# cvxopt/cvxopt

Hardware: NVIDIA H100
Metric: kkt_factor_solve_gflops_fp64 (higher is better)
Workload: dtype f64

## Files before the change

cvxopt_b200/_lib.py:

```python
import ctypes as C
import os

_HERE = os.path.dirname(os.path.abspath(__file__))
LIB_PATH = os.path.join(_HERE, "libcvxopt_b200.so")

HOST, DEVICE = 0, 1
E_ARG, E_CUDA, E_NOMEM, E_NOGPU, E_UNSUP = -1, -2, -3, -4, -5

c_double_p = C.POINTER(C.c_double)
c_int_p = C.POINTER(C.c_int)


class Dims(C.Structure):
    _fields_ = [("mnl", C.c_int), ("ml", C.c_int), ("nq", C.c_int), ("q", c_int_p),
                ("ns", C.c_int), ("s", c_int_p)]


class Scaling(C.Structure):
    _fields_ = [(name, C.c_void_p) for name in
                ("dnl", "dnli", "d", "di", "v", "beta", "r", "rti")]


class SblockArgs(C.Structure):
    _fields_ = ([("nblk", C.c_int), ("orders", C.c_void_p), ("m", C.c_longlong), ("L", C.c_longlong),
# ... 25 lines not shown
    "cvxb_kkt_destroy": (None, [C.c_void_p]),
    "cvxb_kkt_reset": (C.c_int, [C.c_void_p]),
    "cvxb_kkt_set_method": (C.c_int, [C.c_void_p, C.c_int, C.c_double]),
    "cvxb_kkt_set_H": (C.c_int, [C.c_void_p, C.c_void_p, C.c_int, C.c_int]),
    "cvxb_kkt_factor": (C.c_int, [C.c_void_p, C.POINTER(Scaling), C.c_void_p, C.c_int,
                                  C.c_void_p, C.c_int, C.c_int, C.c_int]),
    "cvxb_kkt_solve": (C.c_int, [C.c_void_p, C.c_void_p, C.c_void_p, C.c_void_p, C.c_int]),
    "cvxb_kkt_get_L": (C.c_int, [C.c_void_p, C.c_void_p, C.c_int]),
    "cvxb_kkt_last_ms": (C.c_int, [C.c_void_p, c_double_p, c_double_p]),
    "cvxb_kkt_timer_start": (C.c_int, [C.c_void_p]),
    "cvxb_kkt_timer_stop": (C.c_int, [C.c_void_p, c_double_p]),
    "cvxb_kkt_trace": (C.c_int, [C.c_void_p, C.c_void_p, C.c_int]),
    "cvxb_kkt_last_breakdown": (C.c_int, [C.c_void_p, c_double_p]),
    "cvxb_kkt_syrk_mma_ms": (C.c_int, [C.c_void_p, c_double_p]),
    "cvxb_kkt_syrk_path": (C.c_int, [C.c_void_p]),
    "cvxb_kkt_qr_passes": (C.c_int, [C.c_void_p]),
    "cvxb_kkt_gemv_G": (C.c_int, [C.c_void_p, C.c_void_p, C.c_void_p, C.c_double, C.c_double,
                                  C.c_int, C.c_int]),
    "cvxb_kkt_gemv_A": (C.c_int, [C.c_void_p, C.c_void_p, C.c_void_p, C.c_double, C.c_double,
                                  C.c_int, C.c_int]),
    "cvxb_kkt_symv_H": (C.c_int, [C.c_void_p, C.c_void_p, C.c_void_p, C.c_double, C.c_double,
                                  C.c_int]),
    "cvxb_scale": (C.c_int, [C.c_void_p, C.c_int, C.c_int, C.POINTER(Dims), C.POINTER(Scaling),
                             C.c_int, C.c_int, C.c_int]),
    "cvxb_scale2": (C.c_int, [C.c_void_p, C.c_void_p, C.POINTER(Dims), C.c_int, C.c_int]),
    "cvxb_pack": (C.c_int, [C.c_void_p, C.c_void_p, C.POINTER(Dims), C.c_int]),
    "cvxb_pack2": (C.c_int, [C.c_void_p, C.c_int, C.c_int, C.POINTER(Dims), C.c_int]),
    "cvxb_unpack": (C.c_int, [C.c_void_p, C.c_void_p, C.POINTER(Dims), C.c_int]),
    "cvxb_symm": (C.c_int, [C.c_void_p, C.c_int, C.c_int]),
    "cvxb_sprod": (C.c_int, [C.c_void_p, C.c_void_p, C.POINTER(Dims), C.c_int, C.c_int]),
# ... 123 lines not shown
```

cvxopt_b200/csrc/chol.cu:

```cuda
#include "common.cuh"
#include <cstdlib>

namespace cvxb {

namespace {

constexpr int PB = 8;
constexpr int SP = 12;
constexpr int LDM = NB + 4;
constexpr int POTF2_SMEM = (NB * LDM + NB * SP + 4 * 80) * 8;
constexpr int kGroup = 4;

template <int PAT>
__device__ __forceinline__ void sym_update(double (&acc)[4][8][2], const double *Ma, const double *Mb) {
#pragma unroll 2
    for (int kk = 0; kk < NB / 4; ++kk) {
        double a[4], bfr[8];
#pragma unroll
        for (int cf = 0; cf < 4; ++cf) a[cf] = -Ma[cf * 8 + kk * 4 * LDM];
#pragma unroll
        for (int rf = 0; rf < 8; ++rf) bfr[rf] = Mb[rf * 8 + kk * 4 * LDM];
#pragma unroll
        for (int mf = 0; mf < 2; ++mf)
#pragma unroll
// ... 442 lines not shown
}

std::atomic<int> g_trsv_epoch{0};

__global__ void __launch_bounds__(256)
transpose_panel_kernel(const double *__restrict__ W, long long ldw, int rows, double *__restrict__ WT, long long ldt) {
    __shared__ double t[32][33];
    const int r0 = blockIdx.x * 32, k0 = blockIdx.y * 32, tx = threadIdx.x, ty = threadIdx.y;
#pragma unroll
    for (int i = ty; i < 32; i += 8)
        if (r0 + tx < rows) t[i][tx] = W[r0 + tx + (long long)(k0 + i) * ldw];
    __syncthreads();
#pragma unroll
    for (int i = ty; i < 32; i += 8)
        if (r0 + i < rows) WT[k0 + tx + (long long)(r0 + i) * ldt] = t[tx][i];
}

}

int chol_work_create(CholWork &w) {
    int least = 0, greatest = 0;
    CVXB_CUDA(cudaDeviceGetStreamPriorityRange(&least, &greatest));
    CVXB_CUDA(cudaStreamCreateWithPriority(&w.panel_stream, cudaStreamNonBlocking, greatest));
    CVXB_CUDA(cudaStreamCreateWithPriority(&w.trsm_stream, cudaStreamNonBlocking, greatest));
    CVXB_CUDA(cudaStreamCreateWithPriority(&w.update_stream, cudaStreamNonBlocking, least));
    CVXB_CUDA(cudaStreamCreateWithPriority(&w.near_stream, cudaStreamNonBlocking, greatest));
    CVXB_CUDA(cudaEventCreateWithFlags(&w.ev_end_t, cudaEventDisableTiming));
    CVXB_CUDA(cudaEventCreateWithFlags(&w.ev_end_n, cudaEventDisableTiming));
    CVXB_CUDA(cudaEventCreateWithFlags(&w.ev_start, cudaEventDisableTiming));
    CVXB_CUDA(cudaEventCreateWithFlags(&w.ev_end_p, cudaEventDisableTiming));
// ... 8 lines not shown
    CVXB_CUDA(cudaFuncSetAttribute(trsv_kernel<true, true>, cudaFuncAttributeMaxDynamicSharedMemorySize, TRSV_SMEM));
    CVXB_CUDA(cudaFuncSetAttribute(trsv_kernel<true, false>, cudaFuncAttributeMaxDynamicSharedMemorySize, TRSV_SMEM));
    CVXB_CUDA(cudaFuncSetAttribute(trsv_kernel<false, true>, cudaFuncAttributeMaxDynamicSharedMemorySize, TRSV_SMEM));
    CVXB_CUDA(cudaFuncSetAttribute(trsv_kernel<false, false>, cudaFuncAttributeMaxDynamicSharedMemorySize, TRSV_SMEM));
    return 0;
}

CholWork::~CholWork() {
    for (cudaStream_t s : {panel_stream, update_stream, trsm_stream, near_stream}) if (s) cudaStreamDestroy(s);
    for (auto &g : graphs) if (g.exec) cudaGraphExecDestroy(g.exec);
    for (cudaEvent_t e : {ev_end_t, ev_end_n, ev_start, ev_end_p, ev_end_u}) if (e) cudaEventDestroy(e);
    for (auto *v : {&ev_dg, &ev_tr, &ev_c0, &ev_na, &ev_nb, &ev_n})
        for (cudaEvent_t e : *v) cudaEventDestroy(e);
}

static int potrf_enqueue(int n, double *A, int lda, double *inv, CholWork &w, cudaStream_t st) {
    if (n <= 0) return 0;
    const int nblk = (n + NB - 1) / NB;
    if (w.panel_rows < n) {
        for (auto &g : w.graphs) if (g.exec) cudaGraphExecDestroy(g.exec);
        w.graphs.clear();
        for (DevBuf<double> &pb : w.panel) pb.reset();
        for (DevBuf<double> &gb : w.group) gb.reset();
        const int rows = (n + 1) & ~1;
        for (DevBuf<double> &pb : w.panel) CVXB_TRY(pb.alloc((size_t)rows * NB));
        for (DevBuf<double> &gb : w.group) CVXB_TRY(gb.alloc((size_t)rows * kGroup * NB));
        w.panel_rows = rows;
    }
    while ((int)w.ev_dg.size() < nblk) {
        cudaEvent_t e[6];
        for (int i = 0; i < 6; ++i) CVXB_CUDA(cudaEventCreateWithFlags(&e[i], cudaEventDisableTiming));
        w.ev_dg.push_back(e[0]); w.ev_tr.push_back(e[1]); w.ev_c0.push_back(e[2]);
        w.ev_na.push_back(e[3]); w.ev_nb.push_back(e[4]); w.ev_n.push_back(e[5]);
    }
    if (getenv("CVXB_TRACE") && !w.trace.p) CVXB_TRY(w.trace.alloc(8 * 4096));
    unsigned long long *trace = w.trace.p;
    if (trace) CVXB_CUDA(cudaMemsetAsync(trace, 0, 8 * 4096 * sizeof(unsigned long long), st));
    const int ldw = w.panel_rows;
    const int ldg = kGroup * NB;
    cudaStream_t D = w.panel_stream, T = w.trsm_stream, U = w.update_stream, N = w.near_stream;
    CVXB_CUDA(cudaMemsetAsync(w.d_info.p, 0, sizeof(int), st));
    CVXB_CUDA(cudaEventRecord(w.ev_start, st));
    for (cudaStream_t s : {D, T, U, N}) CVXB_CUDA(cudaStreamWaitEvent(s, w.ev_start, 0));
    auto update = [&](int lo, int hi, const double *X, int ldx, bool kmajor, int K, unsigned long long *tr,
                      cudaStream_t s) -> int {
        double *Acc = A + (long long)lo * NB * (1 + (long long)lda);
        GemmDesc u;
        u.M = n - lo * NB; u.N = (hi * NB < n ? hi * NB : n) - lo * NB; u.K = K;
        u.X = X; u.ldx = ldx; u.x_kmajor = kmajor;
        u.Y = X; u.ldy = ldx; u.y_kmajor = kmajor;
        u.D = Acc; u.ldd = lda; u.C = Acc; u.ldc = lda;
        u.alpha = -1.0; u.beta = 1.0; u.lower_only = true;
        u.trace = tr;
        return dmma_gemm(u, s);
    };
    auto wait_col = [&](cudaStream_t s, int c) -> int {
        const int p = c - 2, g0 = kGroup * (c / kGroup);
        if (p < 0) return 0;
        if (p >= g0) CVXB_CUDA(cudaStreamWaitEvent(s, w.ev_na[p], 0));
        if (g0 > 0) CVXB_CUDA(cudaStreamWaitEvent(s, w.ev_nb[p < g0 - 1 ? p : g0 - 1], 0));
        return 0;
    };
    for (int jb = 0; jb < nblk; ++jb) {
        const int j = jb * NB;
        const int wj = (n - j < NB) ? (n - j) : NB;
        const int m = n - j - wj;
        double *Ajj = A + j + (long long)j * lda;
        double *invj = inv + (long long)jb * NB * NB;
        double *invTj = inv + (long long)(nblk + jb) * NB * NB;
        double *Wp = w.panel[jb & 1].p;
// ... 64 lines not shown
                Wp + (gq - jb - 1) * NB, ldw, rows, Wg + s * NB, ldg);
            count_launch();
            CVXB_LAUNCH_CHECK();
        }
        CVXB_CUDA(cudaEventRecord(w.ev_n[jb], N));
        if (gq < nblk) {
            CVXB_CUDA(cudaStreamWaitEvent(U, w.ev_n[jb], 0));
            const int lo = gq > jb + 2 ? gq : jb + 2, hi = gq + kGroup < nblk ? gq + kGroup : nblk;
            if (lo < hi) CVXB_TRY(update(lo, hi, Wg + s * NB + (long long)(lo - gq) * NB * ldg, ldg, true, NB, tr_near, U));
            CVXB_CUDA(cudaEventRecord(w.ev_nb[jb], U));
            if (s == kGroup - 1 && gq + kGroup < nblk)
                CVXB_TRY(update(gq + kGroup, nblk, Wg + (long long)kGroup * NB * ldg, ldg, true, kGroup * NB,
                                trace ? trace + 8 * 2048 + 8 * jb + 5 : nullptr, U));
        }
    }
    CVXB_CUDA(cudaEventRecord(w.ev_end_p, D));
    CVXB_CUDA(cudaEventRecord(w.ev_end_u, U));
    CVXB_CUDA(cudaEventRecord(w.ev_end_t, T));
    CVXB_CUDA(cudaEventRecord(w.ev_end_n, N));
    for (cudaEvent_t e : {w.ev_end_p, w.ev_end_u, w.ev_end_t, w.ev_end_n}) CVXB_CUDA(cudaStreamWaitEvent(st, e, 0));
    return 0;
}

int potrf_lower(int n, double *A, int lda, double *inv, CholWork &w, cudaStream_t st) {
    if (n <= 0) return 0;
    if (w.graph_failed || n > 4096) return potrf_enqueue(n, A, lda, inv, w, st);
    CholWork::GraphEntry *ent = nullptr;
    for (auto &g : w.graphs)
        if (g.n == n && g.A == A && g.lda == lda && g.inv == inv) { ent = &g; break; }
    if (ent && ent->exec) {
// ... 128 lines not shown
```

cvxopt_b200/csrc/common.cuh:

```cuda
#pragma once
#include <cuda_runtime.h>
#include <cstdio>
#include <cstdint>
#include <cstring>
#include <string>
#include <vector>
#include <atomic>
#include <mutex>
#include "../../include/cvxopt_b200.h"

namespace cvxb {

void set_error(const char *fmt, ...);
extern std::atomic<unsigned long long> g_launches;
inline void count_launch(int n = 1) { g_launches.fetch_add((unsigned long long)n, std::memory_order_relaxed); }

struct DeviceOnce {
    std::atomic<unsigned long long> done{0};
    unsigned long long pending() {
        int d = 0;
        cudaGetDevice(&d);
        const unsigned long long bit = 1ull << (d & 63);
        return (done.load(std::memory_order_acquire) & bit) ? 0ull : bit;
    }
// ... 226 lines not shown

struct GemmDesc {
    int M = 0, N = 0, K = 0;
    const double *X = nullptr; int ldx = 0; bool x_kmajor = false;
    const double *Y = nullptr; int ldy = 0; bool y_kmajor = false;
    const double *w = nullptr;
    const double *D = nullptr; int ldd = 0;
    double *C = nullptr; int ldc = 0;
    double alpha = 1.0, beta = 0.0;
    bool lower_only = false;
    int ct_begin = 0, ct_end = 1 << 30;
    int batch = 1;
    long long sX = 0, sY = 0, sW = 0, sD = 0, sC = 0;
    double *splitk_ws = nullptr;
    unsigned long long *trace = nullptr;
};
int dmma_gemm(const GemmDesc &g, cudaStream_t st);
size_t dmma_gemm_splitk_ws_doubles();
int dmma_gemm_tile_cols();

size_t ozaki_workspace_bytes(int n, int m, int S);
int ozaki_mode();
bool ozaki_use(int mode, int n, int m, DevBuf<char> &work);
void ozaki_time_mma(cudaEvent_t a, cudaEvent_t b);
int ozaki_syrk(int n, int m, const double *A, long long lda, const double *d, const double *D,
               long long ldd, double beta, double *C, long long ldc, int S, int layout, void *work,
               cudaStream_t st);

struct CholWork {
    cudaStream_t panel_stream = nullptr;
// ... 5 lines not shown
    DevBuf<unsigned long long> trace;
    struct GraphEntry {
        int n = 0, lda = 0, launches = 0;
        const void *A = nullptr, *inv = nullptr;
        cudaGraphExec_t exec = nullptr;
    };
    std::vector<GraphEntry> graphs;
    bool graph_failed = false;
    cudaEvent_t ev_start = nullptr, ev_end_p = nullptr, ev_end_u = nullptr;
    DevBuf<int> d_info;
    DevBuf<int> d_flags;
    DevBuf<double> splitk_ws;
    DevBuf<double> panel[2];
    DevBuf<double> group[2];
    int panel_rows = 0;
    ~CholWork();
};
int chol_work_create(CholWork &w);
int potrf_lower(int n, double *A, int lda, double *inv, CholWork &w, cudaStream_t st);
int potrs_lower(int n, const double *L, int ldl, const double *inv, double *b, CholWork &w,
                cudaStream_t st, int batch = 1, long long sL = 0, long long sInv = 0,
                long long sb = 0);
int trsv_lower(int n, const double *L, int ldl, const double *inv, double *b, bool trans,
               CholWork &w, cudaStream_t st, int batch = 1, long long sL = 0, long long sInv = 0,
               long long sb = 0);
int potrf_lower_batched(int n, double *A, int lda, long long sA, double *inv, long long sInv,
                        int batch, int *d_info, double *panel, int ldw, cudaStream_t st);
int trsm_lower_left(int n, const double *L, long long ldl, const double *inv, double *B, long long ldb, int ncols,
                    cudaStream_t st, int batch = 1, long long sL = 0, long long sInv = 0, long long sB = 0);

int check_device(int device);

struct CallCtx {
    cudaStream_t st = nullptr;
// ... 7 lines not shown
```

cvxopt_b200/csrc/gemm_dmma.cu:

```cuda
#include "common.cuh"
#include <cuda.h>
#include <cudaTypedefs.h>

namespace cvxb {

namespace {

constexpr int BR = 128, BC = 64, BK = 16, STAGES = 3;
constexpr int THREADS = 128;
constexpr int SK = BK + 4;
constexpr int SMX = BR + 4;
constexpr int SMY = BC + 4;
constexpr int X_STAGE = BR * SK;
constexpr int Y_STAGE = BC * SK;
constexpr int STAGE_DOUBLES = X_STAGE + Y_STAGE + BK;
constexpr int SMEM_BYTES = STAGES * STAGE_DOUBLES * 8;
constexpr int TILE_ELEMS = BR * BC;
constexpr int CTAS_PER_WAVE = 2 * kNumSMs;
constexpr int SPLITK_WS_TILES = 4 * CTAS_PER_WAVE;

struct KParams {
    int M, N, K;
    const double *X; long long ldx;
    const double *Y; long long ldy;
// ... 1 lines not shown
    const double *D; long long ldd;
    double *C; long long ldc;
    double alpha, beta;
    int lower_only;
    int ct_begin, ct_end;
    int nTr;
    long long sX, sY, sW, sD, sC;
    int full_tiles;
    int S;
    int kchunk;
    double *ws;
    int vec_c;
    int stagger_ns;
    unsigned long long *trace;
    int band;
};

__device__ __host__ __forceinline__ int first_tr(int tc, int tcols) { return (tc * tcols) / BR; }

template <int TC>
__device__ __forceinline__ void decode_tile(const KParams &p, int t, int &tr, int &tc) {
    int c = p.ct_begin;
    if (p.lower_only && p.band > 0) {
        int cb_end;
        while (true) {
            cb_end = min(c + p.band, p.ct_end);
            int cnt = 0;
            for (int cc = c; cc < cb_end; ++cc) cnt += max(0, p.nTr - first_tr(cc, TC));
            if (t < cnt) break;
            t -= cnt;
// ... 357 lines not shown
    }
}

constexpr int TB = 128;
constexpr int T_STAGES = 6;
constexpr int T_CONSUMERS = 8;
constexpr int T_THREADS = 32 * (T_CONSUMERS + 4);
constexpr int T_REGS_PRODUCER = 40, T_REGS_CONSUMER = 232;
constexpr int T_PANEL = TB * BK;
constexpr int T_SMEM = T_STAGES * (2 * T_PANEL + BK) * 8 + 2 * T_STAGES * 8 + 1024;
constexpr int T_TILE_ELEMS = TB * TB;
constexpr int T_WS_TILES = 4 * kNumSMs;

__global__ void __launch_bounds__(T_THREADS, 1)
syrk_tma_kernel(const KParams p, const __grid_constant__ CUtensorMap tmX, const __grid_constant__ CUtensorMap tmY,
                const __grid_constant__ CUtensorMap tmW) {
    extern __shared__ unsigned char t_smem_raw[];
    double *sm = reinterpret_cast<double *>(t_smem_raw + ((1024u - (smem_u32(t_smem_raw) & 1023u)) & 1023u));
    double *sw = sm + T_STAGES * 2 * T_PANEL;
    uint64_t *full = reinterpret_cast<uint64_t *>(sw + T_STAGES * BK), *empty = full + T_STAGES;
    const int tid = threadIdx.x, warp = __shfl_sync(0xffffffffu, tid >> 5, 0), lane = tid & 31;

    const int u = blockIdx.x;
    int tile, split = 0;
    if (u < p.full_tiles) {
        tile = u;
    } else {
        tile = p.full_tiles + (u - p.full_tiles) / p.S;
        split = (u - p.full_tiles) % p.S;
    }
    int tr, tc;
    decode_tile<TB>(p, tile, tr, tc);
    const bool is_split = ((int)blockIdx.x >= p.full_tiles) && (p.S > 1);
    int kbeg = 0, kend = p.K;
    if (is_split) {
        kbeg = split * p.kchunk;
        kend = min(p.K, kbeg + p.kchunk);
// ... 5 lines not shown

    if (tid == 0) {
        for (int s = 0; s < T_STAGES; ++s) { mbar_init(full + s, 1); mbar_init(empty + s, T_CONSUMERS); }
        asm volatile("fence.mbarrier_init.release.cluster;" ::: "memory");
    }
    __syncthreads();

    if (warp >= T_CONSUMERS) {
        asm volatile("setmaxnreg.dec.sync.aligned.u32 %0;" ::"n"(T_REGS_PRODUCER));
        if (warp == T_CONSUMERS && lane == 0) {
            const uint32_t bytes = (uint32_t)(2 * T_PANEL + (has_w ? BK : 0)) * 8u;
            for (int kt = 0; kt < ktiles; ++kt) {
                const int s = kt % T_STAGES;
                if (kt >= T_STAGES) mbar_wait(empty + s, (uint32_t)(kt / T_STAGES - 1) & 1u);
                mbar_expect_tx(full + s, bytes);
                const int k = kbeg + kt * BK;
                tma_load_2d(sm + s * 2 * T_PANEL, &tmX, k, r0, full + s);
                tma_load_2d(sm + s * 2 * T_PANEL + T_PANEL, &tmY, k, c0, full + s);
                if (has_w) tma_load_1d(sw + s * BK, &tmW, k, full + s);
            }
        }
        return;
    }

    asm volatile("setmaxnreg.inc.sync.aligned.u32 %0;" ::"n"(T_REGS_CONSUMER));
    const int wr = warp & 1, wc = warp >> 1;
    const int g4 = lane >> 2, t4 = lane & 3;
    double acc[4][8][2];
    const bool pre_d = p.vec_c && (nr == TB) && (nc == TB) && !(c0 + TB - 1 > r0) && !is_split &&
                       p.beta != 0.0 && p.D != nullptr && (p.alpha == 1.0 || p.alpha == -1.0) && ((p.ldd & 1) == 0);
    if (pre_d) {
        const double sc = p.beta / p.alpha;
        const double *Dt = p.D + r0 + (long long)c0 * p.ldd;
#pragma unroll
// ... 51 lines not shown
#pragma unroll
                    for (int rf = 0; rf < 8; ++rf)
                        dmma16x8x4(acc[2 * mf][rf][0], acc[2 * mf][rf][1], acc[2 * mf + 1][rf][0],
                                   acc[2 * mf + 1][rf][1], a[cur][2 * mf], a[cur][2 * mf + 1], bf[cur][rf]);
                if (kk + 1 == BK / 4 && kt + 1 < ktiles) {
                    const int s1 = (kt + 1) % T_STAGES;
                    mbar_wait(full + s1, (uint32_t)((kt + 1) / T_STAGES) & 1u);
                    load(s1, 0, nxt);
                }
            }
            __syncwarp();
            if (lane == 0) mbar_arrive(empty + s);
        }
    }

    if (is_split) {
        double *ws = p.ws + ((long long)(tile - p.full_tiles) * p.S + split) * T_TILE_ELEMS;
#pragma unroll
        for (int cf = 0; cf < 4; ++cf)
#pragma unroll
            for (int rf = 0; rf < 8; ++rf) {
                const int rl = wr * 64 + rf * 8 + t4 * 2;
                const int cl = wc * 32 + cf * 8 + g4;
                *reinterpret_cast<double2 *>(ws + rl + cl * TB) = make_double2(acc[cf][rf][0], acc[cf][rf][1]);
            }
        return;
    }
    double *C = p.C;
    const double *D = p.D;
    const bool diag = (c0 + TB - 1 > r0);
// ... 111 lines not shown
    const cuuint64_t dims[2] = {(cuuint64_t)K, (cuuint64_t)rows};
    const cuuint64_t strides[1] = {(cuuint64_t)ld * sizeof(double)};
    const cuuint32_t box[2] = {BK, TB};
    const cuuint32_t estr[2] = {1, 1};
    const CUresult r = enc(&m, CU_TENSOR_MAP_DATA_TYPE_FLOAT64, rows ? 2 : 1, const_cast<double *>(base), dims, strides,
                           box, estr, CU_TENSOR_MAP_INTERLEAVE_NONE,
                           rows ? CU_TENSOR_MAP_SWIZZLE_128B : CU_TENSOR_MAP_SWIZZLE_NONE,
                           CU_TENSOR_MAP_L2_PROMOTION_L2_256B, CU_TENSOR_MAP_FLOAT_OOB_FILL_NONE);
    if (r != CUDA_SUCCESS) {
        set_error("dmma_gemm: cuTensorMapEncodeTiled -> CUresult %d", (int)r);
        return CVXB_E_CUDA;
    }
    return 0;
}

int launch_tma(const KParams &p, dim3 grid, cudaStream_t st) {
    CUtensorMap tx, ty, tw;
    CVXB_TRY(encode_operand(tx, p.X, p.ldx, p.K, p.M));
    CVXB_TRY(encode_operand(ty, p.Y, p.ldy, p.K, p.N));
    if (p.w) CVXB_TRY(encode_operand(tw, p.w, 0, p.K, 0));
    else tw = tx;
    static DeviceOnce once;
    if (const unsigned long long bit = once.pending()) {
        CVXB_CUDA(cudaFuncSetAttribute(syrk_tma_kernel, cudaFuncAttributeMaxDynamicSharedMemorySize, T_SMEM));
        once.mark(bit);
    }
    syrk_tma_kernel<<<grid, T_THREADS, T_SMEM, st>>>(p, tx, ty, tw);
    count_launch();
    CVXB_LAUNCH_CHECK();
    return 0;
}

}

size_t dmma_gemm_splitk_ws_doubles() {
    const size_t a = (size_t)SPLITK_WS_TILES * TILE_ELEMS, b = (size_t)T_WS_TILES * T_TILE_ELEMS;
    return a > b ? a : b;
}
int dmma_gemm_tile_cols() { return BC; }

int dmma_gemm(const GemmDesc &g, cudaStream_t st) {
    if (g.M <= 0 || g.N <= 0) return 0;
    if (g.K < 0 || !g.X || !g.Y || !g.C) {
        set_error("dmma_gemm: bad arguments");
        return CVXB_E_ARG;
    }
    auto aligned = [](const void *ptr, long long ld) {
        return ((uintptr_t)ptr % 16 == 0) && (ld % 2 == 0);
    };
    const int nTc = (g.N + BC - 1) / BC;
    const bool tma = g.x_kmajor && g.y_kmajor && g.lower_only && g.batch == 1 && g.K > 0 && g.ct_begin <= 0 &&
                     g.ct_end >= nTc && aligned(g.X, g.ldx) && aligned(g.Y, g.ldy) && ((uintptr_t)g.w % 16 == 0);
    const int tcols = tma ? TB : BC;
    const int wave = tma ? kNumSMs : CTAS_PER_WAVE;
    KParams p;
    p.M = g.M; p.N = g.N; p.K = g.K;
    p.X = g.X; p.ldx = g.ldx; p.Y = g.Y; p.ldy = g.ldy; p.w = g.w;
    p.D = g.D; p.ldd = g.ldd; p.C = g.C; p.ldc = g.ldc;
    p.alpha = g.alpha; p.beta = (g.D ? g.beta : 0.0);
    p.lower_only = g.lower_only ? 1 : 0;
    p.nTr = (g.M + BR - 1) / BR;
    p.ct_begin = g.ct_begin < 0 ? 0 : g.ct_begin;
    p.ct_end = g.ct_end > nTc ? nTc : g.ct_end;
    if (p.ct_begin >= p.ct_end) return 0;
    if (tma) p.ct_end = (g.N + TB - 1) / TB;
    p.sX = g.sX; p.sY = g.sY; p.sW = g.sW; p.sD = g.sD; p.sC = g.sC;
    p.band = (p.lower_only && g.K >= 1024 && g.batch == 1) ? 1024 / tcols : 0;
    long long T = 0;
    if (p.lower_only) {
        for (int c = p.ct_begin; c < p.ct_end; ++c) {
            int cnt = p.nTr - first_tr(c, tcols);
            T += cnt > 0 ? cnt : 0;
        }
    } else {
        T = (long long)p.nTr * (p.ct_end - p.ct_begin);
    }
    if (T <= 0) return 0;
    p.full_tiles = (int)T; p.S = 1; p.kchunk = g.K; p.ws = nullptr;
    if (g.splitk_ws && g.batch == 1 && g.K >= 1024) {
        int full = (int)(T / wave) * wave;
        int rem = (int)T - full;
        if (rem > 0) {
            int maxS = g.K / 512;
            if (maxS > 18) maxS = 18;
            const int cap_units = tma ? T_WS_TILES : SPLITK_WS_TILES;
            int bestS = 1;
            double best = 1.0;
            for (int S = 2; S <= maxS; ++S) {
                if ((long long)rem * S > cap_units) break;
                const double cost = (double)((rem * S + wave - 1) / wave) / S;
                if (cost < best - 1e-9) { best = cost; bestS = S; }
            }
            if (bestS >= 2) {
                p.full_tiles = full;
                p.S = bestS;
                int kc = (g.K + bestS - 1) / bestS;
                p.kchunk = ((kc + BK - 1) / BK) * BK;
                p.ws = g.splitk_ws;
            }
        }
    }
    p.stagger_ns = 0;
    p.trace = g.trace;
    if (!tma && g.K <= 512 && T > CTAS_PER_WAVE) p.stagger_ns = ((g.K + BK - 1) / BK) * 1050;
    const int rem_tiles = (int)T - p.full_tiles;
    const int units = p.full_tiles + rem_tiles * p.S;
    dim3 grid(units, 1, g.batch);
    const bool vec = aligned(g.X, g.ldx) && aligned(g.Y, g.ldy) &&
                     (g.batch == 1 || (g.sX % 2 == 0 && g.sY % 2 == 0));
    p.vec_c = aligned(g.C, g.ldc) && (!g.D || aligned(g.D, g.ldd)) &&
              (g.batch == 1 || (g.sC % 2 == 0 && g.sD % 2 == 0));
    int rc;
#define DISPATCH(XK, YK)                                                   \
    rc = vec ? launch_inst<XK, YK, true>(p, grid, st) : launch_inst<XK, YK, false>(p, grid, st)
    if (tma) rc = launch_tma(p, grid, st);
    else if (g.x_kmajor && g.y_kmajor) DISPATCH(true, true);
    else if (g.x_kmajor && !g.y_kmajor) DISPATCH(true, false);
    else if (!g.x_kmajor && g.y_kmajor) DISPATCH(false, true);
    else DISPATCH(false, false);
#undef DISPATCH
    if (rc) return rc;
    if (p.S > 1) {
        dim3 rg(rem_tiles, 8);
        if (tma) splitk_reduce_kernel<TB><<<rg, 256, 0, st>>>(p);
        else splitk_reduce_kernel<BC><<<rg, 256, 0, st>>>(p);
        count_launch();
        CVXB_LAUNCH_CHECK();
    }
    return 0;
}
// ... 3 lines not shown
```

cvxopt_b200/csrc/kkt_api.cu:

```cuda
#include "cone.cuh"
#include <cstdlib>
#include <cstdarg>
#include <map>
#include <unordered_map>
#include <mutex>
#include <iterator>

namespace cvxb {

static thread_local std::string g_err;
std::atomic<unsigned long long> g_launches{0};
std::atomic<unsigned long long> g_device_bytes{0};


namespace {
struct TmpCache {
    std::mutex mu;
    std::multimap<size_t, void *> free_[64];
    std::unordered_map<void *, std::pair<size_t, int>> live;
    size_t cached = 0, cap = 0;
    bool cap_set = false;
};
TmpCache &tmpc() { static TmpCache *c = new TmpCache; return *c; }
size_t tmp_round(size_t b) { return b <= 4096 ? 4096 : (b + 65535) & ~(size_t)65535; }
// ... 386 lines not shown
    if (!k) { set_error("kkt is NULL"); return CVXB_E_ARG; }
    CVXB_CUDA(cudaSetDevice(k->device));
    if (!H) {
        k->Hres.reset();
        return 0;
    }
    if (ldh < (k->n > 1 ? k->n : 1)) { set_error("set_H: ldh < n"); return CVXB_E_ARG; }
    const long long ldk = kkt_ldk(k);
    if (!k->Hres.p) CVXB_TRY(k->Hres.alloc((size_t)ldk * (k->n > 0 ? k->n : 1)));
    CVXB_TRY(upload_matrix(k->Hres.p, ldk, H, ldh, k->n, k->n, space, k->st));
    CVXB_TRY(symmetrize_lower(k->n, k->Hres.p, ldk, 1, 0, k->st));
    CVXB_CUDA(cudaStreamSynchronize(k->st));
    return 0;
}

int cvxb_kkt_factor(cvxb_kkt *k, const cvxb_scaling *Wp, const double *H, int ldh,
                    const double *Df, int lddf, int use_resident_H, int space) {
    if (!k) { set_error("kkt is NULL"); return CVXB_E_ARG; }
    CVXB_CUDA(cudaSetDevice(k->device));
    if (k->method == 1) {
        if (H || Df || k->cone.mnl) { set_error("kkt_qr: the QR route solves systems with a zero (1,1) block (no H, no Df)"); return CVXB_E_ARG; }
        k->factored = false;
        int r = kkt_qr_factor(k, Wp, space);
        k->factored = (r == 0);
        return r;
    }
    const ConeLayout &c = k->cone;
    const int n = k->n;
    cudaStream_t st = k->st;
    k->factored = false;
// ... 30 lines not shown
        bool have = false;
        auto syrk_add = [&](const double *X, long long ldx, int kdim, const double *w) -> int {
            GemmDesc g;
            g.M = n; g.N = n; g.K = kdim;
            g.X = X; g.ldx = (int)ldx; g.x_kmajor = true;
            g.Y = X; g.ldy = (int)ldx; g.y_kmajor = true;
            g.w = w;
            g.D = have ? K : Hptr; g.ldd = have ? (int)ldk : (int)ldH; g.beta = 1.0;
            g.C = K; g.ldc = (int)ldk;
            g.lower_only = true; g.splitk_ws = k->cw.splitk_ws.p;
            CVXB_TRY(dmma_gemm(g, st));
            have = true;
            return 0;
        };
        k->syrk_path = 0;
        if (c.ml > 0 && n > 0 && ozaki_use(k->i8_mode, n, c.ml, k->oz_work)) {
            ozaki_time_mma(k->m0, k->m1);
            CVXB_TRY(ozaki_syrk(n, c.ml, k->G + c.mnl, k->ldg, k->W.di, Hptr, ldH, 1.0, K, ldk, 9, 0,
                                k->oz_work.p, st));
            have = true;
            k->syrk_path = 2;
        } else if (c.ml > 0 && n > 0) {
            CVXB_TRY(syrk_add(k->G + c.mnl, k->ldg, c.ml, k->W.di2));
            k->syrk_path = 1;
        }
        if (k->nrest > 0 && n > 0) CVXB_TRY(syrk_add(k->Gs.p, k->ldgs, k->nrest, nullptr));
        if (add_ata && k->p > 0 && n > 0) CVXB_TRY(syrk_add(k->Aeq.p, k->lda_eq, k->p, nullptr));
        if (!have && n > 0) {
            if (!Hptr) { set_error("factor: no cone rows and no H: KKT matrix is singular"); return 1; }
            CVXB_TRY(upload_matrix(K, ldk, Hptr, ldH, n, n, CVXB_DEVICE, st));
        }
// ... 107 lines not shown
    if (!k || !ms) return CVXB_E_ARG;
    CVXB_CUDA(cudaSetDevice(k->device));
    CVXB_CUDA(cudaEventRecord(k->t1, k->st));
    CVXB_CUDA(cudaEventSynchronize(k->t1));
    float t = 0;
    CVXB_CUDA(cudaEventElapsedTime(&t, k->t0, k->t1));
    *ms = t;
    return 0;
}
int cvxb_kkt_trace(cvxb_kkt *k, unsigned long long *out, int nsteps) {
    if (!k || !out || !k->cw.trace.p) return CVXB_E_ARG;
    CVXB_CUDA(cudaMemcpy(out, k->cw.trace.p, (size_t)nsteps * 8 * sizeof(unsigned long long), cudaMemcpyDeviceToHost));
    return 0;
}
int cvxb_kkt_syrk_path(cvxb_kkt *k) { return k ? k->syrk_path : CVXB_E_ARG; }
int cvxb_kkt_qr_passes(cvxb_kkt *k) { return (k && k->method == 1) ? k->qr->npass : CVXB_E_ARG; }
int cvxb_kkt_last_breakdown(cvxb_kkt *k, double *ms3) {
    if (!k || !ms3) return CVXB_E_ARG;
    ms3[0] = k->br[1]; ms3[1] = k->br[2]; ms3[2] = k->br[0];
    return 0;
}

int cvxb_kkt_syrk_mma_ms(cvxb_kkt *k, double *ms) {
    if (!k || !ms) return CVXB_E_ARG;
    *ms = k->mma_ms;
    return 0;
}

int cvxb_kkt_gemv_G(cvxb_kkt *k, const double *x, double *y, double alpha, double beta, int trans,
                    int space) {
// ... 66 lines not shown
```

cvxopt_b200/csrc/kkt_internal.cuh:

```cuda
#pragma once
#include "cone.cuh"
#include <memory>

using cvxb::ConeLayout;
using cvxb::DevScaling;
using cvxb::CholWork;
using cvxb::DevBuf;

namespace cvxb {
struct QrState {
    int nq = 0;
    DevBuf<double> Q;
    long long ldQ = 0;
    DevBuf<double> R1;
    DevBuf<double> tau;
    DevBuf<double> GsF;
    DevBuf<double> GsQ;
    long long ldf = 0;
    DevBuf<double> Q3t;
    long long ldq = 0;
    DevBuf<double> C[3], inv[3];
    long long ldc = 0;
    int npass = 2;
    DevBuf<double> w, u, vv, xt, ws, norm2;
// ... 39 lines not shown
    bool first_factor = true;
    DevScaling W;
    DevBuf<double> bzp, zin, zt, xv, yv;
    DevBuf<double> gemv_ws;
    DevBuf<double> swork;
    CholWork cw;
    cudaStream_t st = nullptr;
    cudaEvent_t e0 = nullptr, e1 = nullptr, e2 = nullptr, e3 = nullptr, t0 = nullptr, t1 = nullptr;
    cudaEvent_t m0 = nullptr, m1 = nullptr;
    double mma_ms = 0.0;
    double factor_ms = 0, solve_ms = 0, br[3] = {0, 0, 0};
    bool factored = false;
    int i8_mode = 0;
    DevBuf<char> oz_work;
    int syrk_path = 0;
    int method = 0;
    std::unique_ptr<cvxb::QrState> qr;
    std::unique_ptr<cvxb::LdlState> ldl;
    ~cvxb_kkt();
};


namespace cvxb {
int upload_matrix(double *dst, long long ldd, const double *src, long long lds, int rows, int cols, int space,
                  cudaStream_t st);
int xfer_vec(double *dst, const double *src, size_t n, int space, bool to_device, cudaStream_t st);
inline long long kkt_ldk(const cvxb_kkt *k) { long long l = (k->n + 1) & ~1; return l > 2 ? l : 2; }
int kkt_pack_bz(cvxb_kkt *k, const double *zd);
int kkt_unpack_z(cvxb_kkt *k, double *zd);
int kkt_scale_pack_G(cvxb_kkt *k, double *dst, long long ldd);
// ... 8 lines not shown
```

cvxopt_b200/kkt.py:

```python
import ctypes as C

import numpy as np

from . import _lib


def _mat(a, name="matrix"):
    arr = np.asarray(a)
    if arr.dtype != np.float64:
        if arr.dtype.kind in "iuf":
            arr = arr.astype(np.float64)
        else:
            raise TypeError("%s must be a real 'd' matrix" % name)
    if arr.ndim == 1:
        arr = arr.reshape(-1, 1)
    if arr.ndim != 2:
        raise TypeError("%s must be two-dimensional" % name)
    if not arr.flags.f_contiguous:
        arr = np.asfortranarray(arr)
    return arr


def _vec_inplace(a, n, name):
    arr = np.asarray(a)
# ... 205 lines not shown
        return f.value, s.value

    def last_breakdown(self):
        b = (C.c_double * 3)()
        self._lib.cvxb_kkt_last_breakdown(self._h, b)
        out = {"syrk_ms": b[0], "potrf_ms": b[1], "scale_ms": b[2]}
        mm = C.c_double()
        self._lib.cvxb_kkt_syrk_mma_ms(self._h, C.byref(mm))
        if mm.value > 0:
            out["syrk_mma_ms"] = mm.value
        return out

    def syrk_path(self):
        return ("none", "dmma", "int8")[self._lib.cvxb_kkt_syrk_path(self._h)]

    def qr_passes(self):
        return self._lib.cvxb_kkt_qr_passes(self._h)

    def get_L(self):
        L = np.zeros((self.n, self.n), order="F")
        _lib.check(self._lib.cvxb_kkt_get_L(self._h, L.ctypes.data, max(1, self.n)), "get_L")
        return np.tril(L)

    def close(self):
        if getattr(self, "_h", None) is not None and self._h.value:
            self._lib.cvxb_kkt_destroy(self._h)
            self._h = C.c_void_p()

    def __del__(self):
        try:
# ... 43 lines not shown
```

include/cvxopt_b200.h:

```cpp
#ifndef CVXOPT_B200_H
#define CVXOPT_B200_H

#ifdef __cplusplus
extern "C" {
#endif

#define CVXB_E_ARG     (-1)
#define CVXB_E_CUDA    (-2)
#define CVXB_E_NOMEM   (-3)
#define CVXB_E_NOGPU   (-4)
#define CVXB_E_UNSUP   (-5)

#define CVXB_HOST   0
#define CVXB_DEVICE 1

typedef struct cvxb_kkt cvxb_kkt;
typedef struct cvxb_batch cvxb_batch;

typedef struct {
    int mnl;
    int ml;
    int nq;
    const int *q;
    int ns;
// ... 30 lines not shown

int cvxb_kkt_set_H(cvxb_kkt *k, const double *H, int ldh, int space);

int cvxb_kkt_factor(cvxb_kkt *k, const cvxb_scaling *W, const double *H, int ldh,
                    const double *Df, int lddf, int use_resident_H, int space);

int cvxb_kkt_solve(cvxb_kkt *k, double *x, double *y, double *z, int space);

int cvxb_kkt_get_L(cvxb_kkt *k, double *L_host, int ldl);
int cvxb_kkt_last_ms(cvxb_kkt *k, double *factor_ms, double *solve_ms);
int cvxb_kkt_timer_start(cvxb_kkt *k);
int cvxb_kkt_timer_stop(cvxb_kkt *k, double *ms);
int cvxb_kkt_trace(cvxb_kkt *k, unsigned long long *out, int nsteps);
int cvxb_kkt_last_breakdown(cvxb_kkt *k, double *ms3);
int cvxb_kkt_syrk_path(cvxb_kkt *k);
int cvxb_kkt_syrk_mma_ms(cvxb_kkt *k, double *ms);
int cvxb_kkt_qr_passes(cvxb_kkt *k);

int cvxb_kkt_gemv_G(cvxb_kkt *k, const double *x, double *y, double alpha, double beta,
                    int trans, int space);
int cvxb_kkt_symv_H(cvxb_kkt *k, const double *x, double *y, double alpha, double beta,
                    int space);
int cvxb_kkt_gemv_A(cvxb_kkt *k, const double *x, double *y, double alpha, double beta,
                    int trans, int space);


int cvxb_scale(double *x, int xr, int xc, const cvxb_dims *dims, const cvxb_scaling *W,
               int trans , int inverse , int space);
int cvxb_scale2(const double *lmbda, double *x, const cvxb_dims *dims, int inverse,
                int space);
// ... 129 lines not shown
```

Before: 40140.

## Fuse SYRK formation with blocked Cholesky in left-looking superpanel pipeline

```diff
diff --git a/cvxopt_b200/_lib.py b/cvxopt_b200/_lib.py
--- a/cvxopt_b200/_lib.py
+++ b/cvxopt_b200/_lib.py
@@ -63,6 +63,7 @@
     "cvxb_kkt_last_breakdown": (C.c_int, [C.c_void_p, c_double_p]),
     "cvxb_kkt_syrk_mma_ms": (C.c_int, [C.c_void_p, c_double_p]),
     "cvxb_kkt_syrk_path": (C.c_int, [C.c_void_p]),
+    "cvxb_kkt_factor_route": (C.c_int, [C.c_void_p]),
     "cvxb_kkt_qr_passes": (C.c_int, [C.c_void_p]),
     "cvxb_kkt_gemv_G": (C.c_int, [C.c_void_p, C.c_void_p, C.c_void_p, C.c_double, C.c_double,
                                   C.c_int, C.c_int]),
diff --git a/cvxopt_b200/csrc/chol.cu b/cvxopt_b200/csrc/chol.cu
--- a/cvxopt_b200/csrc/chol.cu
+++ b/cvxopt_b200/csrc/chol.cu
@@ -480,6 +480,11 @@
 #pragma unroll
     for (int i = ty; i < 32; i += 8)
         if (r0 + i < rows) WT[k0 + tx + (long long)(r0 + i) * ldt] = t[tx][i];
+}
+
+__global__ void fill_kernel(double *x, int n, double v) {
+    const int i = blockIdx.x * blockDim.x + threadIdx.x;
+    if (i < n) x[i] = v;
 }
 
 }
@@ -518,8 +523,7 @@
         for (cudaEvent_t e : *v) cudaEventDestroy(e);
 }
 
-static int potrf_enqueue(int n, double *A, int lda, double *inv, CholWork &w, cudaStream_t st) {
-    if (n <= 0) return 0;
+static int chol_buffers(int n, CholWork &w) {
     const int nblk = (n + NB - 1) / NB;
     if (w.panel_rows < n) {
         for (auto &g : w.graphs) if (g.exec) cudaGraphExecDestroy(g.exec);
@@ -538,6 +542,26 @@
         w.ev_na.push_back(e[3]); w.ev_nb.push_back(e[4]); w.ev_n.push_back(e[5]);
     }
     if (getenv("CVXB_TRACE") && !w.trace.p) CVXB_TRY(w.trace.alloc(8 * 4096));
+    return 0;
+}
+
+static int trailing_update(int n, double *A, int lda, int lo, int hi, const double *X, int ldx, bool kmajor, int K,
+                           unsigned long long *tr, cudaStream_t s) {
+    double *Acc = A + (long long)lo * NB * (1 + (long long)lda);
+    GemmDesc u;
+    u.M = n - lo * NB; u.N = (hi * NB < n ? hi * NB : n) - lo * NB; u.K = K;
+    u.X = X; u.ldx = ldx; u.x_kmajor = kmajor;
+    u.Y = X; u.ldy = ldx; u.y_kmajor = kmajor;
+    u.D = Acc; u.ldd = lda; u.C = Acc; u.ldc = lda;
+    u.alpha = -1.0; u.beta = 1.0; u.lower_only = true;
+    u.trace = tr;
+    return dmma_gemm(u, s);
+}
+
+static int potrf_enqueue(int n, double *A, int lda, double *inv, CholWork &w, cudaStream_t st) {
+    if (n <= 0) return 0;
+    const int nblk = (n + NB - 1) / NB;
+    CVXB_TRY(chol_buffers(n, w));
     unsigned long long *trace = w.trace.p;
     if (trace) CVXB_CUDA(cudaMemsetAsync(trace, 0, 8 * 4096 * sizeof(unsigned long long), st));
     const int ldw = w.panel_rows;
@@ -547,17 +571,7 @@
     CVXB_CUDA(cudaEventRecord(w.ev_start, st));
     for (cudaStream_t s : {D, T, U, N}) CVXB_CUDA(cudaStreamWaitEvent(s, w.ev_start, 0));
     auto update = [&](int lo, int hi, const double *X, int ldx, bool kmajor, int K, unsigned long long *tr,
-                      cudaStream_t s) -> int {
-        double *Acc = A + (long long)lo * NB * (1 + (long long)lda);
-        GemmDesc u;
-        u.M = n - lo * NB; u.N = (hi * NB < n ? hi * NB : n) - lo * NB; u.K = K;
-        u.X = X; u.ldx = ldx; u.x_kmajor = kmajor;
-        u.Y = X; u.ldy = ldx; u.y_kmajor = kmajor;
-        u.D = Acc; u.ldd = lda; u.C = Acc; u.ldc = lda;
-        u.alpha = -1.0; u.beta = 1.0; u.lower_only = true;
-        u.trace = tr;
-        return dmma_gemm(u, s);
-    };
+                      cudaStream_t s) -> int { return trailing_update(n, A, lda, lo, hi, X, ldx, kmajor, K, tr, s); };
     auto wait_col = [&](cudaStream_t s, int c) -> int {
         const int p = c - 2, g0 = kGroup * (c / kGroup);
         if (p < 0) return 0;
@@ -652,6 +666,139 @@
                                 trace ? trace + 8 * 2048 + 8 * jb + 5 : nullptr, U));
         }
     }
+    CVXB_CUDA(cudaEventRecord(w.ev_end_p, D));
+    CVXB_CUDA(cudaEventRecord(w.ev_end_u, U));
+    CVXB_CUDA(cudaEventRecord(w.ev_end_t, T));
+    CVXB_CUDA(cudaEventRecord(w.ev_end_n, N));
+    for (cudaEvent_t e : {w.ev_end_p, w.ev_end_u, w.ev_end_t, w.ev_end_n}) CVXB_CUDA(cudaStreamWaitEvent(st, e, 0));
+    return 0;
+}
+
+int potrf_formed(int n, double *A, int lda, double *inv, const double *G, int ldg, int m, const double *wg,
+                 const double *H, int ldh, CholWork &w, cudaStream_t st, cudaEvent_t formed) {
+    if (n <= 0) return 0;
+    constexpr int kS = kFormedPanel / NB;
+    const int nblk = (n + NB - 1) / NB, nsup = (nblk + kS - 1) / kS;
+    CVXB_TRY(chol_buffers(n, w));
+    if ((int)w.neg_ones.n < n) {
+        w.neg_ones.reset();
+        CVXB_TRY(w.neg_ones.alloc((size_t)n));
+        fill_kernel<<<(n + 255) / 256, 256, 0, st>>>(w.neg_ones.p, n, -1.0);
+        count_launch();
+        CVXB_LAUNCH_CHECK();
+    }
+    unsigned long long *trace = w.trace.p;
+    if (trace) CVXB_CUDA(cudaMemsetAsync(trace, 0, 8 * 4096 * sizeof(unsigned long long), st));
+    const int ldw = w.panel_rows;
+    cudaStream_t D = w.panel_stream, T = w.trsm_stream, U = w.update_stream, N = w.near_stream;
+    CVXB_CUDA(cudaMemsetAsync(w.d_info.p, 0, sizeof(int), st));
+    CVXB_CUDA(cudaEventRecord(w.ev_start, st));
+    for (cudaStream_t s : {D, T, U, N}) CVXB_CUDA(cudaStreamWaitEvent(s, w.ev_start, 0));
+    auto form = [&](int s, int k2) -> int {
+        const int c0 = s * kFormedPanel, c1 = c0 + kFormedPanel < n ? c0 + kFormedPanel : n;
+        GemmDesc g;
+        g.M = n - c0; g.N = c1 - c0; g.K = m;
+        g.X = G + (long long)c0 * ldg; g.ldx = ldg; g.x_kmajor = true;
+        g.Y = g.X; g.ldy = ldg; g.y_kmajor = true;
+        g.w = wg;
+        g.X2 = A + (long long)c0 * lda; g.ldx2 = lda;
+        g.Y2 = g.X2; g.ldy2 = lda;
+        g.w2 = w.neg_ones.p; g.K2 = k2;
+        g.D = H ? H + c0 + (long long)c0 * ldh : nullptr; g.ldd = ldh; g.beta = 1.0;
+        g.C = A + c0 + (long long)c0 * lda; g.ldc = lda;
+        g.lower_only = true; g.splitk_ws = w.splitk_ws.p;
+        g.trace = trace ? trace + 8 * 3072 + 4 * s : nullptr;
+        return dmma_gemm(g, U);
+    };
+    CVXB_TRY(form(0, 0));
+    for (int s = 0; s < nsup; ++s) {
+        const int b0 = s * kS, b1 = b0 + kS < nblk ? b0 + kS : nblk;
+        if (s > 0) {
+            CVXB_CUDA(cudaStreamWaitEvent(U, w.ev_n[b0 - 1], 0));
+            CVXB_TRY(trailing_update(n, A, lda, b0, b1, A + (long long)(b0 - kS) * NB + (long long)b0 * NB * lda, lda,
+                                     true, kFormedPanel, trace ? trace + 8 * 3072 + 4 * s + 2 : nullptr, U));
+        }
+        CVXB_CUDA(cudaEventRecord(w.ev_nb[s], U));
+        if (s + 1 < nsup) CVXB_TRY(form(s + 1, b0 * NB));
+        for (int jb = b0; jb < b1; ++jb) {
+            const int j = jb * NB;
+            const int wj = (n - j < NB) ? (n - j) : NB;
+            const int mr = n - j - wj;
+            double *Ajj = A + j + (long long)j * lda;
+            double *invj = inv + (long long)jb * NB * NB;
+            double *invTj = inv + (long long)(nblk + jb) * NB * NB;
+            double *Wp = w.panel[jb & 1].p;
+            if (jb == b0) {
+                CVXB_CUDA(cudaStreamWaitEvent(D, w.ev_nb[s], 0));
+            } else if (jb - 2 >= b0) {
+                CVXB_CUDA(cudaStreamWaitEvent(D, w.ev_c0[jb - 2], 0));
+                CVXB_CUDA(cudaStreamWaitEvent(D, w.ev_na[jb - 2], 0));
+            }
+            const double *Tprev = jb > b0 ? A + j + (long long)(j - NB) * lda : nullptr;
+            const double *invprev = jb > b0 ? inv + (long long)(jb - 1) * NB * NB : nullptr;
+            potf2_inv_kernel<<<1, 256, POTF2_SMEM, D>>>(Ajj, lda, wj, invj, invTj, w.d_info.p, j, 0, 0, Tprev,
+                                                         lda, invprev, trace ? trace + 8 * jb : nullptr);
+            count_launch();
+            CVXB_LAUNCH_CHECK();
+            CVXB_CUDA(cudaEventRecord(w.ev_dg[jb], D));
+            auto copy_back = [&](int pb) -> int {
+                const int jp = pb * NB, rows = n - jp - NB;
+                CVXB_CUDA(cudaMemcpy2DAsync(A + jp + NB + (long long)jp * lda, (size_t)lda * sizeof(double),
+                                            w.panel[pb & 1].p, (size_t)ldw * sizeof(double),
+                                            (size_t)rows * sizeof(double), NB, cudaMemcpyDeviceToDevice, T));
+                return 0;
+            };
+            if (mr <= 0) {
+                CVXB_CUDA(cudaStreamWaitEvent(T, w.ev_dg[jb], 0));
+                if (jb > b0) CVXB_TRY(copy_back(jb - 1));
+                break;
+            }
+            double *A21 = Ajj + wj;
+            double *A22 = A21 + (long long)wj * lda;
+            CVXB_CUDA(cudaStreamWaitEvent(T, w.ev_dg[jb], 0));
+            if (jb >= 2) CVXB_CUDA(cudaStreamWaitEvent(T, w.ev_n[jb - 2], 0));
+            {
+                GemmDesc g;
+                g.M = mr; g.N = wj; g.K = wj;
+                g.X = A21; g.ldx = lda; g.x_kmajor = false;
+                g.Y = invj; g.ldy = NB; g.y_kmajor = false;
+                g.C = Wp; g.ldc = ldw;
+                g.trace = trace ? trace + 8 * jb + 2 : nullptr;
+                CVXB_TRY(dmma_gemm(g, T));
+            }
+            CVXB_CUDA(cudaEventRecord(w.ev_tr[jb], T));
+            const int wn = (mr < NB) ? mr : NB;
+            if (jb + 1 < b1 && mr > wn) {
+                if (jb - 1 >= b0) CVXB_CUDA(cudaStreamWaitEvent(T, w.ev_na[jb - 1], 0));
+                GemmDesc c;
+                c.M = mr - wn; c.N = wn; c.K = wj;
+                c.X = Wp + wn; c.Y = Wp;
+                c.ldx = ldw; c.x_kmajor = false;
+                c.ldy = ldw; c.y_kmajor = false;
+                c.D = A22 + wn; c.ldd = lda; c.C = A22 + wn; c.ldc = lda;
+                c.alpha = -1.0; c.beta = 1.0;
+                c.trace = trace ? trace + 8 * jb + 4 : nullptr;
+                CVXB_TRY(dmma_gemm(c, T));
+            }
+            CVXB_CUDA(cudaEventRecord(w.ev_c0[jb], T));
+            if (jb > b0) CVXB_TRY(copy_back(jb - 1));
+            if (jb + 1 == b1) CVXB_TRY(copy_back(jb));
+            CVXB_CUDA(cudaStreamWaitEvent(N, w.ev_tr[jb], 0));
+            if (jb + 2 < b1)
+                CVXB_TRY(trailing_update(n, A, lda, jb + 2, b1, Wp + NB, ldw, false, NB,
+                                         trace ? trace + 8 * jb + 6 : nullptr, N));
+            CVXB_CUDA(cudaEventRecord(w.ev_na[jb], N));
+            if (b1 < nblk) {
+                const int rows = n - b1 * NB;
+                transpose_panel_kernel<<<dim3((rows + 31) / 32, NB / 32), dim3(32, 8), 0, N>>>(
+                    Wp + (b1 - jb - 1) * NB, ldw, rows, A + j + (long long)b1 * NB * lda, lda);
+                count_launch();
+                CVXB_LAUNCH_CHECK();
+            }
+            CVXB_CUDA(cudaEventRecord(w.ev_n[jb], N));
+        }
+    }
+    CVXB_CUDA(cudaEventRecord(formed, U));
     CVXB_CUDA(cudaEventRecord(w.ev_end_p, D));
     CVXB_CUDA(cudaEventRecord(w.ev_end_u, U));
     CVXB_CUDA(cudaEventRecord(w.ev_end_t, T));
diff --git a/cvxopt_b200/csrc/common.cuh b/cvxopt_b200/csrc/common.cuh
--- a/cvxopt_b200/csrc/common.cuh
+++ b/cvxopt_b200/csrc/common.cuh
@@ -264,6 +264,10 @@
     long long sX = 0, sY = 0, sW = 0, sD = 0, sC = 0;
     double *splitk_ws = nullptr;
     unsigned long long *trace = nullptr;
+    const double *X2 = nullptr; int ldx2 = 0;
+    const double *Y2 = nullptr; int ldy2 = 0;
+    const double *w2 = nullptr;
+    int K2 = 0;
 };
 int dmma_gemm(const GemmDesc &g, cudaStream_t st);
 size_t dmma_gemm_splitk_ws_doubles();
@@ -299,10 +303,14 @@
     DevBuf<double> panel[2];
     DevBuf<double> group[2];
     int panel_rows = 0;
+    DevBuf<double> neg_ones;
     ~CholWork();
 };
 int chol_work_create(CholWork &w);
 int potrf_lower(int n, double *A, int lda, double *inv, CholWork &w, cudaStream_t st);
+constexpr int kFormedPanel = 512;
+int potrf_formed(int n, double *A, int lda, double *inv, const double *G, int ldg, int m, const double *wg,
+                 const double *H, int ldh, CholWork &w, cudaStream_t st, cudaEvent_t formed);
 int potrs_lower(int n, const double *L, int ldl, const double *inv, double *b, CholWork &w,
                 cudaStream_t st, int batch = 1, long long sL = 0, long long sInv = 0,
                 long long sb = 0);
diff --git a/cvxopt_b200/csrc/gemm_dmma.cu b/cvxopt_b200/csrc/gemm_dmma.cu
--- a/cvxopt_b200/csrc/gemm_dmma.cu
+++ b/cvxopt_b200/csrc/gemm_dmma.cu
@@ -39,6 +39,7 @@
     int stagger_ns;
     unsigned long long *trace;
     int band;
+    int kseg;
 };
 
 __device__ __host__ __forceinline__ int first_tr(int tc, int tcols) { return (tc * tcols) / BR; }
@@ -426,13 +427,18 @@
 
 __global__ void __launch_bounds__(T_THREADS, 1)
 syrk_tma_kernel(const KParams p, const __grid_constant__ CUtensorMap tmX, const __grid_constant__ CUtensorMap tmY,
-                const __grid_constant__ CUtensorMap tmW) {
+                const __grid_constant__ CUtensorMap tmW, const __grid_constant__ CUtensorMap tmX2,
+                const __grid_constant__ CUtensorMap tmY2, const __grid_constant__ CUtensorMap tmW2) {
     extern __shared__ unsigned char t_smem_raw[];
     double *sm = reinterpret_cast<double *>(t_smem_raw + ((1024u - (smem_u32(t_smem_raw) & 1023u)) & 1023u));
     double *sw = sm + T_STAGES * 2 * T_PANEL;
     uint64_t *full = reinterpret_cast<uint64_t *>(sw + T_STAGES * BK), *empty = full + T_STAGES;
     const int tid = threadIdx.x, warp = __shfl_sync(0xffffffffu, tid >> 5, 0), lane = tid & 31;
 
+    if (p.trace && tid == 0) {
+        unsigned long long t; asm volatile("mov.u64 %0, %%globaltimer;" : "=l"(t));
+        atomicCAS(p.trace, 0ULL, t);
+    }
     const int u = blockIdx.x;
     int tile, split = 0;
     if (u < p.full_tiles) {
@@ -468,10 +474,11 @@
                 const int s = kt % T_STAGES;
                 if (kt >= T_STAGES) mbar_wait(empty + s, (uint32_t)(kt / T_STAGES - 1) & 1u);
                 mbar_expect_tx(full + s, bytes);
-                const int k = kbeg + kt * BK;
-                tma_load_2d(sm + s * 2 * T_PANEL, &tmX, k, r0, full + s);
-                tma_load_2d(sm + s * 2 * T_PANEL + T_PANEL, &tmY, k, c0, full + s);
-                if (has_w) tma_load_1d(sw + s * BK, &tmW, k, full + s);
+                const bool seg2 = kbeg + kt * BK >= p.kseg;
+                const int k = kbeg + kt * BK - (seg2 ? p.kseg : 0);
+                tma_load_2d(sm + s * 2 * T_PANEL, seg2 ? &tmX2 : &tmX, k, r0, full + s);
+                tma_load_2d(sm + s * 2 * T_PANEL + T_PANEL, seg2 ? &tmY2 : &tmY, k, c0, full + s);
+                if (has_w) tma_load_1d(sw + s * BK, seg2 ? &tmW2 : &tmW, k, full + s);
             }
         }
         return;
@@ -553,6 +560,10 @@
         }
     }
 
+    if (p.trace && tid == 0) {
+        unsigned long long t; asm volatile("mov.u64 %0, %%globaltimer;" : "=l"(t));
+        atomicMax(p.trace + 1, t);
+    }
     if (is_split) {
         double *ws = p.ws + ((long long)(tile - p.full_tiles) * p.S + split) * T_TILE_ELEMS;
 #pragma unroll
@@ -694,18 +705,26 @@
     return 0;
 }
 
-int launch_tma(const KParams &p, dim3 grid, cudaStream_t st) {
-    CUtensorMap tx, ty, tw;
-    CVXB_TRY(encode_operand(tx, p.X, p.ldx, p.K, p.M));
-    CVXB_TRY(encode_operand(ty, p.Y, p.ldy, p.K, p.N));
-    if (p.w) CVXB_TRY(encode_operand(tw, p.w, 0, p.K, 0));
+int launch_tma(const KParams &p, const GemmDesc &g, dim3 grid, cudaStream_t st) {
+    CUtensorMap tx, ty, tw, tx2, ty2, tw2;
+    CVXB_TRY(encode_operand(tx, p.X, p.ldx, g.K, p.M));
+    CVXB_TRY(encode_operand(ty, p.Y, p.ldy, g.K, p.N));
+    if (p.w) CVXB_TRY(encode_operand(tw, p.w, 0, g.K, 0));
     else tw = tx;
+    if (g.K2 > 0) {
+        CVXB_TRY(encode_operand(tx2, g.X2, g.ldx2, g.K2, p.M));
+        CVXB_TRY(encode_operand(ty2, g.Y2, g.ldy2, g.K2, p.N));
+        if (g.w2) CVXB_TRY(encode_operand(tw2, g.w2, 0, g.K2, 0));
+        else tw2 = tx;
+    } else {
+        tx2 = tx; ty2 = ty; tw2 = tw;
+    }
     static DeviceOnce once;
     if (const unsigned long long bit = once.pending()) {
         CVXB_CUDA(cudaFuncSetAttribute(syrk_tma_kernel, cudaFuncAttributeMaxDynamicSharedMemorySize, T_SMEM));
         once.mark(bit);
     }
-    syrk_tma_kernel<<<grid, T_THREADS, T_SMEM, st>>>(p, tx, ty, tw);
+    syrk_tma_kernel<<<grid, T_THREADS, T_SMEM, st>>>(p, tx, ty, tw, tx2, ty2, tw2);
     count_launch();
     CVXB_LAUNCH_CHECK();
     return 0;
@@ -729,12 +748,21 @@
         return ((uintptr_t)ptr % 16 == 0) && (ld % 2 == 0);
     };
     const int nTc = (g.N + BC - 1) / BC;
+    const bool seg2 = g.K2 > 0;
     const bool tma = g.x_kmajor && g.y_kmajor && g.lower_only && g.batch == 1 && g.K > 0 && g.ct_begin <= 0 &&
-                     g.ct_end >= nTc && aligned(g.X, g.ldx) && aligned(g.Y, g.ldy) && ((uintptr_t)g.w % 16 == 0);
+                     g.ct_end >= nTc && aligned(g.X, g.ldx) && aligned(g.Y, g.ldy) && ((uintptr_t)g.w % 16 == 0) &&
+                     (!seg2 || (aligned(g.X2, g.ldx2) && aligned(g.Y2, g.ldy2) && ((uintptr_t)g.w2 % 16 == 0) &&
+                                (g.w == nullptr) == (g.w2 == nullptr)));
+    if (seg2 && !tma) {
+        set_error("dmma_gemm: a second K segment needs the TMA kernel's operands (K-major, lower, 16-byte aligned)");
+        return CVXB_E_ARG;
+    }
+    const int Ktot = seg2 ? (g.K + BK - 1) / BK * BK + g.K2 : g.K;
     const int tcols = tma ? TB : BC;
     const int wave = tma ? kNumSMs : CTAS_PER_WAVE;
     KParams p;
-    p.M = g.M; p.N = g.N; p.K = g.K;
+    p.M = g.M; p.N = g.N; p.K = Ktot;
+    p.kseg = seg2 ? Ktot - g.K2 : Ktot;
     p.X = g.X; p.ldx = g.ldx; p.Y = g.Y; p.ldy = g.ldy; p.w = g.w;
     p.D = g.D; p.ldd = g.ldd; p.C = g.C; p.ldc = g.ldc;
     p.alpha = g.alpha; p.beta = (g.D ? g.beta : 0.0);
@@ -745,7 +773,7 @@
     if (p.ct_begin >= p.ct_end) return 0;
     if (tma) p.ct_end = (g.N + TB - 1) / TB;
     p.sX = g.sX; p.sY = g.sY; p.sW = g.sW; p.sD = g.sD; p.sC = g.sC;
-    p.band = (p.lower_only && g.K >= 1024 && g.batch == 1) ? 1024 / tcols : 0;
+    p.band = (p.lower_only && Ktot >= 1024 && g.batch == 1) ? 1024 / tcols : 0;
     long long T = 0;
     if (p.lower_only) {
         for (int c = p.ct_begin; c < p.ct_end; ++c) {
@@ -756,12 +784,12 @@
         T = (long long)p.nTr * (p.ct_end - p.ct_begin);
     }
     if (T <= 0) return 0;
-    p.full_tiles = (int)T; p.S = 1; p.kchunk = g.K; p.ws = nullptr;
-    if (g.splitk_ws && g.batch == 1 && g.K >= 1024) {
+    p.full_tiles = (int)T; p.S = 1; p.kchunk = Ktot; p.ws = nullptr;
+    if (g.splitk_ws && g.batch == 1 && Ktot >= 1024) {
         int full = (int)(T / wave) * wave;
         int rem = (int)T - full;
         if (rem > 0) {
-            int maxS = g.K / 512;
+            int maxS = Ktot / 512;
             if (maxS > 18) maxS = 18;
             const int cap_units = tma ? T_WS_TILES : SPLITK_WS_TILES;
             int bestS = 1;
@@ -774,7 +802,7 @@
             if (bestS >= 2) {
                 p.full_tiles = full;
                 p.S = bestS;
-                int kc = (g.K + bestS - 1) / bestS;
+                int kc = (Ktot + bestS - 1) / bestS;
                 p.kchunk = ((kc + BK - 1) / BK) * BK;
                 p.ws = g.splitk_ws;
             }
@@ -793,7 +821,7 @@
     int rc;
 #define DISPATCH(XK, YK)                                                   \
     rc = vec ? launch_inst<XK, YK, true>(p, grid, st) : launch_inst<XK, YK, false>(p, grid, st)
-    if (tma) rc = launch_tma(p, grid, st);
+    if (tma) rc = launch_tma(p, g, grid, st);
     else if (g.x_kmajor && g.y_kmajor) DISPATCH(true, true);
     else if (g.x_kmajor && !g.y_kmajor) DISPATCH(true, false);
     else if (!g.x_kmajor && g.y_kmajor) DISPATCH(false, true);
diff --git a/cvxopt_b200/csrc/kkt_api.cu b/cvxopt_b200/csrc/kkt_api.cu
--- a/cvxopt_b200/csrc/kkt_api.cu
+++ b/cvxopt_b200/csrc/kkt_api.cu
@@ -424,6 +424,8 @@
     return 0;
 }
 
+static constexpr int kFormedMinN = 4096;
+
 int cvxb_kkt_factor(cvxb_kkt *k, const cvxb_scaling *Wp, const double *H, int ldh,
                     const double *Df, int lddf, int use_resident_H, int space) {
     if (!k) { set_error("kkt is NULL"); return CVXB_E_ARG; }
@@ -484,7 +486,20 @@
             return 0;
         };
         k->syrk_path = 0;
-        if (c.ml > 0 && n > 0 && ozaki_use(k->i8_mode, n, c.ml, k->oz_work)) {
+        k->formed = false;
+        const bool i8 = c.ml > 0 && n > 0 && ozaki_use(k->i8_mode, n, c.ml, k->oz_work);
+        const double *Gl = k->G + c.mnl;
+        if (!i8 && k->method == 0 && c.ml > 0 && k->nrest == 0 && !(add_ata && k->p > 0) && n >= kFormedMinN &&
+            (uintptr_t)Gl % 16 == 0 && k->ldg % 2 == 0 && (uintptr_t)k->W.di2 % 16 == 0) {
+            k->syrk_path = 1;
+            k->formed = true;
+            CVXB_TRY(potrf_formed(n, K, (int)ldk, k->inv.p, Gl, (int)k->ldg, c.ml, k->W.di2, Hptr, (int)ldH, k->cw, st,
+                                  k->e2));
+            CVXB_CUDA(cudaMemcpyAsync(&info, k->cw.d_info.p, sizeof(int), cudaMemcpyDeviceToHost, st));
+            CVXB_CUDA(cudaStreamSynchronize(st));
+            return 0;
+        }
+        if (i8) {
             ozaki_time_mma(k->m0, k->m1);
             CVXB_TRY(ozaki_syrk(n, c.ml, k->G + c.mnl, k->ldg, k->W.di, Hptr, ldH, 1.0, K, ldk, 9, 0,
                                 k->oz_work.p, st));
@@ -622,6 +637,7 @@
     return 0;
 }
 int cvxb_kkt_syrk_path(cvxb_kkt *k) { return k ? k->syrk_path : CVXB_E_ARG; }
+int cvxb_kkt_factor_route(cvxb_kkt *k) { return k ? (k->formed ? 1 : 0) : CVXB_E_ARG; }
 int cvxb_kkt_qr_passes(cvxb_kkt *k) { return (k && k->method == 1) ? k->qr->npass : CVXB_E_ARG; }
 int cvxb_kkt_last_breakdown(cvxb_kkt *k, double *ms3) {
     if (!k || !ms3) return CVXB_E_ARG;
diff --git a/cvxopt_b200/csrc/kkt_internal.cuh b/cvxopt_b200/csrc/kkt_internal.cuh
--- a/cvxopt_b200/csrc/kkt_internal.cuh
+++ b/cvxopt_b200/csrc/kkt_internal.cuh
@@ -77,6 +77,7 @@
     int i8_mode = 0;
     DevBuf<char> oz_work;
     int syrk_path = 0;
+    bool formed = false;
     int method = 0;
     std::unique_ptr<cvxb::QrState> qr;
     std::unique_ptr<cvxb::LdlState> ldl;
diff --git a/cvxopt_b200/kkt.py b/cvxopt_b200/kkt.py
--- a/cvxopt_b200/kkt.py
+++ b/cvxopt_b200/kkt.py
@@ -243,6 +243,9 @@
     def syrk_path(self):
         return ("none", "dmma", "int8")[self._lib.cvxb_kkt_syrk_path(self._h)]
 
+    def factor_route(self):
+        return ("two-phase", "formed")[self._lib.cvxb_kkt_factor_route(self._h)]
+
     def qr_passes(self):
         return self._lib.cvxb_kkt_qr_passes(self._h)
 
diff --git a/include/cvxopt_b200.h b/include/cvxopt_b200.h
--- a/include/cvxopt_b200.h
+++ b/include/cvxopt_b200.h
@@ -68,6 +68,7 @@
 int cvxb_kkt_trace(cvxb_kkt *k, unsigned long long *out, int nsteps);
 int cvxb_kkt_last_breakdown(cvxb_kkt *k, double *ms3);
 int cvxb_kkt_syrk_path(cvxb_kkt *k);
+int cvxb_kkt_factor_route(cvxb_kkt *k);
 int cvxb_kkt_syrk_mma_ms(cvxb_kkt *k, double *ms);
 int cvxb_kkt_qr_passes(cvxb_kkt *k);
 
```

After: 40960, median of 6. +2.0%, better.
